# Cryptum169/another-cuda-sift

Hardware: AMD Instinct MI355X
Metric: detectAndCompute Mpix/s + 2kx2k 128-D match ms at 1/2/4/8 MI355X (higher is better)
Workload: dtype f32; 1 GPU; C2: detectAndCompute on 1920x1200 frames, 16 per step per GPU (one launch per stage for the batch), numOctaveLayers=3 (5 DoG scales/octave), numOctaves=3, upscale=false, numFeatures=5000; frames HBM-resident; frames_per_launch=16, streams_per_gpu=2, parallelism=frame-sharded x1, no data-path collective, descriptor_mode=fixed-point (default), keypoints_per_frame=4366

## Files before the change

### another-cuda-sift_amd/csrc/detector.hip

```cpp
#include <hip/hip_runtime.h>

#include <algorithm>
#include <cmath>
#include <cstdio>

#include "detector_state.h"

namespace sift_amd {
namespace det {

thread_local std::string g_err;

int fail(int code, const std::string& msg) {
    g_err = msg;
    return code;
}

namespace {

int gaussian_ntaps(double sigma) { return (int)lrint(sigma * 4 * 2 + 1) | 1; }

Taps gaussian_taps(double sigma) {
    Taps t{};
    const int n = gaussian_ntaps(sigma);
// ... 101 lines not shown
            snprintf(msg, sizeof msg,
                     "sigma %g with numOctaveLayers %d gives a layer blur of one tap (its sigma %g < 0.0625); "
                     "the smallest kernel has 3 taps",
                     d->cfg.sigma, L, sig[i]);
            return fail(SIFT_HIP_ERR_INVALID, msg);
        }
    d->initTaps = gaussian_taps((double)sig_diff);
    d->layerTaps.assign(L + 3, Taps{});
    for (int i = 1; i < L + 3; i++) d->layerTaps[i] = gaussian_taps(sig[i]);
    d->tailOct = L + 3 <= kTailMaxPlanes ? tail_first_octave(d->pyr, d->layerTaps.data(), L) : d->nOct;
    d->threshold = (float)(int)std::floor(0.5 * d->cfg.contrastThreshould / L * 255 * 1.0);
    d->kp.contrastThreshold = (float)d->cfg.contrastThreshould;
    d->kp.edgeThreshold = (float)d->cfg.edgeThreshould;
    d->kp.sigma = (float)d->cfg.sigma;
    d->kp.numFeatures = d->cfg.numFeatures;
    double sumPx = 0;
    for (int o = 0; o < d->nOct; o++) sumPx += (double)d->pyr.oct[o].W * d->pyr.oct[o].H;
    auto clampu = [](double v, double lo, double hi) { return (unsigned)std::max(lo, std::min(v, hi)); };
    d->capCand = clampu(sumPx * L / 8, 16384, 1u << 20);
    d->kp.capRefined = std::min(d->capCand, 1u << 18);
    d->kp.capOriented = 2 * d->kp.capRefined;
    const int nfeat = d->cfg.numFeatures;
    d->kp.capFinal = d->cfg.maxKeypoints > 0 ? (unsigned)d->cfg.maxKeypoints
                     : nfeat > 0             ? clampu(nfeat + std::max(nfeat / 4, 512), 1024, 65536)
                                             : clampu(sumPx / 32, 4096, 65536);
    const double sclMax = d->cfg.sigma * std::pow(2.0, (L + 0.5) / L);
    d->kp.oriRmax = (int)lrint(4.5 * sclMax) + 1;
    d->kp.descRmax = std::min((int)lrint(3.0 * sclMax * 1.4142135623730951 * 2.5) + 1, 60);
    const double hw = 3.0 * sclMax;
    d->kp.descNrec = std::min((int)std::ceil((5.0 * hw + 3.0) * (5.0 * hw + 3.0)), 8192);
    return SIFT_HIP_OK;
}

void upload_exp_tab() {
    const double A0 = .9670371139572337719125840413672004409288e-2;
    float tab[64];
    for (int j = 0; j < 64; j++) tab[j] = (float)(std::exp2((double)j / 64.0) * A0);
    upload_exp_table(tab);
    upload_desc_exp_table(tab);
}

void bind_lane(sift_hip_detector* d, int k, int idx) {
    Lane& L = d->lanes[k];
    const ArenaLayout& a = d->lay;
    char* A = L.arena;
    d->ln = k;
    d->stream = L.stream;
    d->dInput = reinterpret_cast<float*>(A + a.input);
    d->dUp = d->firstOctave < 0 ? reinterpret_cast<float*>(A + a.up) : nullptr;
    d->dPyr = reinterpret_cast<float*>(A + a.pyr);
    for (int o = 0; o < d->nOct; o++) d->pyr.oct[o].base = d->dPyr + a.octave[o];
    d->dCand = reinterpret_cast<uint2*>(A + a.cand);
    d->dRef = reinterpret_cast<RefKpt*>(A + a.ref);
    d->dOri = reinterpret_cast<OriKpt*>(A + a.ori);
    d->dSlot = reinterpret_cast<int*>(A + a.slot);
    d->dOrder = reinterpret_cast<int*>(A + a.order);
    d->dJobs = reinterpret_cast<DescJob*>(A + a.jobs);
    d->dJord = reinterpret_cast<JobOrder*>(A + a.jord);
    d->dRange = reinterpret_cast<unsigned*>(A + a.range);
    d->dBcount = reinterpret_cast<unsigned*>(A + a.bcount);
    d->dBoff = reinterpret_cast<unsigned*>(A + a.boff);
    d->dBitmap = reinterpret_cast<uint32_t*>(A + a.bitmap);
    d->dCtr = reinterpret_cast<Counters*>(A + a.ctr);
    char* R = A + (size_t)idx * d->afs;
    for (int b = 0; b < d->kSlots; b++) {
        d->dKpts3[b] = reinterpret_cast<float*>(R + a.k3[b]);
        d->dFeats4[b] = reinterpret_cast<float*>(R + a.f4[b]);
        d->dDesc[b] = reinterpret_cast<uint16_t*>(R + a.desc[b]);
        d->dSide[b] = Sidecar{reinterpret_cast<int8_t*>(R + a.codes[b]), reinterpret_cast<int*>(R + a.ckeys[b])};
    }
    d->hCtr = L.hCtr + idx;
    d->hCtrDev = L.hCtrDev + idx;
}

const uint16_t* frame_desc(const sift_hip_detector* d, long long f) {
    const auto& r = d->frecs[f & (kFrameRing - 1)];
    return reinterpret_cast<const uint16_t*>(d->lanes[r.lane].arena + (size_t)r.idx * d->afs + d->lay.desc[r.slot]);
}
const Counters& frame_counters(const sift_hip_detector* d, long long f, int i) {
    const auto& r = d->frecs[f & (kFrameRing - 1)];
    return d->lanes[r.lane].hCtr[(size_t)r.slot * d->lanes[r.lane].B + r.idx + i];
}

int allocate(sift_hip_detector* d) {
    HIPCHK(hipSetDevice(d->device));
    d->allocated = true;
    if (d->tailOct < d->nOct) {
        int optin = 0;
        if (hipDeviceGetAttribute(&optin, hipDeviceAttributeSharedMemPerBlockOptin, d->device) != hipSuccess ||
            optin < (int)(sizeof(float) * kTailLdsFloats) || tail_init() != hipSuccess) {
            (void)hipGetLastError();
            d->tailOct = d->nOct;
        }
    }
    HIPCHK(hipEventCreateWithFlags(&d->evIn, hipEventDisableTiming));
    HIPCHK(hipEventCreateWithFlags(&d->evOut, hipEventDisableTiming));
    const int W = d->cfg.col_width, H = d->cfg.row_width;
    d->inPitch = (W + 63) / 64 * 64;
    if (d->firstOctave < 0) d->upPitch = (2 * W + 63) / 64 * 64;
    size_t pyrFloats = 0;
    for (int o = 0; o < d->nOct; o++) pyrFloats += (size_t)d->pyr.oct[o].planeStride * (d->L + 3);
    const unsigned capO = d->kp.capOriented, capF = d->kp.capFinal;

    size_t off = 0;
    auto take = [&](size_t bytes) {
        const size_t o = off;
        off += (std::max<size_t>(bytes, 1) + 255) & ~(size_t)255;
        return o;
    };
    ArenaLayout& a = d->lay;
    a.input = take(sizeof(float) * (size_t)d->inPitch * H);
    a.up = d->firstOctave < 0 ? take(sizeof(float) * (size_t)d->upPitch * 2 * H) : 0;
    a.pyr = take(sizeof(float) * pyrFloats);
    a.cand = take(sizeof(uint2) * d->capCand);
    a.ref = take(sizeof(RefKpt) * d->kp.capRefined);
    a.ori = take(sizeof(OriKpt) * capO);
    a.slot = take(sizeof(int) * capO);
    a.order = take(sizeof(int) * capO);
    a.jobs = take(sizeof(DescJob) * capF);
    a.jord = take(sizeof(JobOrder));
    a.range = take(sizeof(unsigned) * 2 * 2 * kRangeSlots);
    a.bcount = take(sizeof(unsigned) * (size_t)d->kp.numBuckets);
    a.boff = take(sizeof(unsigned) * (size_t)d->kp.numBuckets);
    a.bitmap = take(sizeof(uint32_t) * d->bitmapWords);
    a.ctr = take(sizeof(Counters));
    for (int b = 0; b < d->kSlots; b++) {
        a.k3[b] = take(sizeof(float) * 3 * (size_t)capF);
        a.f4[b] = take(sizeof(float) * 4 * (size_t)capF);
        a.desc[b] = take(sizeof(uint16_t) * 128 * (size_t)capF);
        a.codes[b] = take(128 * (size_t)capF);
        a.ckeys[b] = take(sizeof(int) * (size_t)capF);
    }
    d->afs = (long)off;
    upload_exp_tab();
    return SIFT_HIP_OK;
}

int build_graphs(sift_hip_detector* d);

int add_lane(sift_hip_detector* d, int B, int nslots) {
    if (d->nLanes >= kMaxLanes) return fail(SIFT_HIP_ERR_STATE, "no lane left");
    const int k = d->nLanes;
    Lane& L = d->lanes[k];
    d->nLanes++;
    L.B = B;
    L.nslots = nslots;
    HIPCHK(hipStreamCreateWithFlags(&L.stream, hipStreamNonBlocking));
    if (hipMalloc((void**)&L.arena, (size_t)d->afs * B) != hipSuccess)
        return fail(SIFT_HIP_ERR_NOMEM, "hipMalloc of the frame arenas failed");
    HIPCHK(hipMemsetAsync(L.arena, 0, (size_t)d->afs * B, L.stream));
    const size_t nh = (size_t)nslots * B;
    HIPCHK(hipHostMalloc((void**)&L.hCtr, sizeof(Counters) * nh, hipHostMallocMapped | hipHostMallocCoherent));
    memset(L.hCtr, 0, sizeof(Counters) * nh);
    HIPCHK(hipHostGetDevicePointer((void**)&L.hCtrDev, L.hCtr, 0));
    if (hipMalloc((void**)&L.dHostTab, sizeof(char*) * nh) != hipSuccess)
        return fail(SIFT_HIP_ERR_NOMEM, "hipMalloc of the host results table failed");
    HIPCHK(hipMemsetAsync(L.dHostTab, 0, sizeof(char*) * nh, L.stream));
    for (int b = 0; b < d->kSlots; b++) {
        HIPCHK(hipEventCreateWithFlags(&L.evFrame[b], hipEventDisableTiming));
        HIPCHK(hipEventRecord(L.evFrame[b], L.stream));
    }
    std::fill(std::begin(L.hostFrame), std::end(L.hostFrame), -1LL);
    const size_t inBytes = sizeof(float) * (size_t)d->inPitch * d->cfg.row_width;
    for (int i = 0; i < Lane::kInSlots; i++) {
        HIPCHK(hipHostMalloc(&L.hStage[i], inBytes, hipHostMallocMapped | hipHostMallocNonCoherent));
        HIPCHK(hipEventCreateWithFlags(&L.evRead[i], hipEventDisableTiming));
        HIPCHK(hipEventRecord(L.evRead[i], L.stream));
    }
    bind_lane(d, k);
    for (int i = 0; i < B; i++)
        for (int b = 0; b < d->kSlots; b++)
            register_sidecar(d, fptr(d->dDesc[b], (long)i * d->afs),
                             Sidecar{fptr(d->dSide[b].codes, (long)i * d->afs), fptr(d->dSide[b].keys, (long)i * d->afs)},
                             (int)d->kp.capFinal);
    if (d->hostWant)
        if (int rc = ensure_host_res(d, L)) return rc;
    if (int rc = build_graphs(d)) return rc;
    L.ready = true;
    return SIFT_HIP_OK;
}

unsigned* range_keys(sift_hip_detector* d, int p) { return d->dRange + (size_t)p * 2 * kRangeSlots; }

void enqueue_head(sift_hip_detector* d, const void* img, int pitch, int fmt, int parity, int nf, long sfs) {
    const int W = d->cfg.col_width, H = d->cfg.row_width;
    const bool u8 = fmt == SIFT_HIP_U8;
    const Frames fr{nf, d->afs};
    const double inB = (double)W * H * (u8 ? 1 : 4) * nf;
    if (d->firstOctave < 0) {
        d->timed("upsample", inB + (double)W * H * 16 * nf, [&] {
            if (u8)
                launch_upsample2x_u8((const uint8_t*)img, pitch, W, H, d->dUp, d->upPitch, fr, sfs, d->stream);
            else
                launch_upsample2x((const float*)img, pitch, W, H, d->dUp, d->upPitch, fr, sfs, d->stream);
        });
    } else {
        const OctGeom& g = d->pyr.oct[0];
        d->timed("blur_init", inB + (double)W * H * 4 * nf, [&] {
            long s = sfs;
            if (u8) {
                if (launch_blur_u8((const uint8_t*)img, pitch, W, H, g.base, g.pitch, d->initTaps, fr, sfs, d->stream,
                                   range_keys(d, parity), d->dCtr))
                    return;
                launch_u8_to_f32((const uint8_t*)img, pitch, W, H, d->dInput, d->inPitch, fr, sfs, d->stream);
                img = d->dInput;
                pitch = d->inPitch;
                s = d->afs;
            }
            launch_blur((const float*)img, pitch, W, H, g.base, g.pitch, DecOut{}, d->initTaps, fr, s, d->stream,
                        range_keys(d, parity), d->dCtr);
        });
    }
}

void left_tail(sift_hip_detector* d, int nf, hipStream_t s) {
    if (d->tailOct >= d->nOct) return;
    double bytes = 0;
    for (int o = d->tailOct; o < d->nOct; o++)
        bytes += (double)d->pyr.oct[o].W * d->pyr.oct[o].H * 4 * (o == d->tailOct ? 1 + (d->L + 2) : (d->L + 2)) * nf;
    d->timed("pyr_tail", bytes, [&] { launch_blur_tail(d->pyr, d->layerTaps.data(), d->L, d->tailOct, Frames{nf, d->afs}, s); });
}

void enqueue_pyramid(sift_hip_detector* d, int nf, int parity) {
    hipStream_t s = d->stream;
    const int L = d->L;
    const Frames fr{nf, d->afs};
    if (d->firstOctave < 0) {
        const OctGeom& g = d->pyr.oct[0];
        d->timed("blur_init", (double)g.W * g.H * 8 * nf, [&] {
            launch_blur(d->dUp, d->upPitch, g.W, g.H, g.base, g.pitch, DecOut{}, d->initTaps, fr, d->afs, s,
                        range_keys(d, parity), d->dCtr);
        });
    }
    static const char* blurNames[kMaxOctaves] = {"blur_o0", "blur_o1", "blur_o2", "blur_o3", "blur_o4", "blur_o5",
                                                 "blur_o6", "blur_o7", "blur_o8", "blur_o9", "blur_o10", "blur_o11",
                                                 "blur_o12", "blur_o13", "blur_o14", "blur_o15"};
    struct Job {
        int o, i;
        BlurDesc b;
        double bytes;
    };
    std::vector<Job> jobs;
    for (int o = 0; o < d->tailOct; o++) {
        const OctGeom& g = d->pyr.oct[o];
        for (int i = 1; i < L + 3; i++) {
            Job j{o, i, {}, 0};
            j.b.src = g.base + (size_t)(i - 1) * g.planeStride;
            j.b.spitch = g.pitch;
            j.b.dst = g.base + (size_t)i * g.planeStride;
            j.b.dpitch = g.pitch;
            j.b.W = g.W;
            j.b.H = g.H;
            j.b.taps = &d->layerTaps[i];
            j.bytes = (double)g.W * g.H * 8 * nf;
            if (i == L && o + 1 < d->nOct) {
                const OctGeom& n = d->pyr.oct[o + 1];
                j.b.dec = DecOut{n.base, n.pitch, n.W, n.H};
                j.bytes += (double)n.W * n.H * 4 * nf;
            }
            jobs.push_back(j);
        }
    }
    auto idx = [&](int o, int i) { return o * (L + 2) + (i - 1); };
    std::vector<bool> done(jobs.size(), false);
    auto ready = [&](size_t k) {
        const Job& j = jobs[k];
        if (done[k]) return false;
        if (j.i >= 2) return (bool)done[idx(j.o, j.i - 1)];
        return j.o == 0 || (bool)done[idx(j.o - 1, L)];
    };
    if (jobs.empty()) left_tail(d, nf, s);
    for (size_t left = jobs.size(); left > 0;) {
        int a = -1, b = -1;
        for (size_t k = 0; k < jobs.size() && b < 0; k++)
            if (ready(k)) (a < 0 ? a : b) = (int)k;
        const Job& ja = jobs[a];
        bool paired = false;
        if (b >= 0) {
            const Job& jb = jobs[b];
            char name[16];
            snprintf(name, sizeof name, "blur_o%d+o%d", ja.o, jb.o);
            d->timed(name, ja.bytes + jb.bytes, [&] { paired = launch_blur_pair(ja.b, jb.b, fr, s); });
            if (paired) {
                done[b] = true;
                left--;
            }
        }
        if (!paired) {
            d->timed(blurNames[ja.o], ja.bytes, [&] {
                launch_blur(ja.b.src, ja.b.spitch, ja.b.W, ja.b.H, ja.b.dst, ja.b.dpitch, ja.b.dec,
                            *ja.b.taps, fr, d->afs, s);
            });
        }
        done[a] = true;
        left--;
    }
    if (!jobs.empty()) left_tail(d, nf, s);
}

void enqueue_extrema(sift_hip_detector* d, int nf) {
    hipStream_t s = d->stream;
    const int L = d->L;
    const Frames fr{nf, d->afs};
    double exBytes = 0;
    for (int o = 0; o < d->nOct; o++) exBytes += (double)d->pyr.oct[o].W * d->pyr.oct[o].H * 4 * (L + 3) * nf;
    d->timed("extrema", exBytes, [&] {
        if (!launch_extrema_all(d->pyr, d->threshold, d->dCand, d->dCtr, d->capCand, fr, s))
            for (int o = 0; o < d->nOct; o++)
                launch_extrema(d->pyr, o, d->threshold, d->dCand, d->dCtr, d->capCand, fr, s);
    });
}

void enqueue_refine(sift_hip_detector* d, int nf) {
    const Frames fr{nf, d->afs};
    d->timed("refine", 0, [&] {
        launch_refine(d->pyr, d->dCand, d->capCand, d->dCtr, d->dBitmap, d->dRef, d->kp, fr, d->stream);
    });
}

void enqueue_orientation(sift_hip_detector* d, int nf, const MaskArg& mask) {
    const Frames fr{nf, d->afs};
    d->timed("orientation", 0,
             [&] { launch_orientation(d->pyr, d->dRef, d->dCtr, d->dOri, d->dBitmap, d->kp, fr, d->stream, mask); });
}

void enqueue_order(sift_hip_detector* d, int slot, int nf, const MaskArg& mask) {
    hipStream_t s = d->stream;
    const int parity = slot & 1;
    const Frames fr{nf, d->afs};
    if (d->kp.numBuckets <= kOrderMaxBuckets) {
        d->timed("order", 0, [&] {
            launch_order(d->pyr, d->dOri, d->dCtr, range_keys(d, parity ^ 1), d->dBcount, d->dBoff, d->dSlot, d->dOrder,
                         d->dJord, d->kp, fr, s, mask);
        });
    } else {
        d->timed("select", 0, [&] { launch_select(d->dOri, d->dCtr, range_keys(d, parity ^ 1), d->kp, fr, s); });
        d->timed("bucket_count", 0,
                 [&] { launch_bucket_count(d->dOri, d->dCtr, d->dBcount, d->dSlot, d->kp, fr, s, mask); });
        d->timed("bucket_scan", 0, [&] { launch_bucket_scan(d->dBcount, d->dBoff, d->dCtr, d->kp, fr, s); });
        d->timed("bucket_scatter", 0,
                 [&] { launch_bucket_scatter(d->dOri, d->dCtr, d->dBoff, d->dSlot, d->dOrder, d->kp, fr, s); });
    }
    d->timed("bucket_rank", 0, [&] {
        if (d->kp.numBuckets <= kOrderMaxBuckets)
            launch_rank_final(d->pyr, d->dOri, d->dBcount, d->dBoff, d->dOrder, d->dCtr, d->dJord, d->dJobs, d->dKpts3[slot],
                              d->dFeats4[slot], d->kp, fr, s);
        else
            launch_bucket_rank(d->pyr, d->dOri, d->dBcount, d->dBoff, d->dOrder, d->dCtr, d->dJobs, d->dKpts3[slot],
                               d->dFeats4[slot], d->kp, fr, s);
    });
}

void enqueue_descriptor(sift_hip_detector* d, int slot, int nf) {
    const Frames fr{nf, d->afs};
    d->timed("descriptor", 0, [&] {
        launch_descriptor(d->dJobs, d->dCtr, range_keys(d, slot & 1), d->dDesc[slot], d->dSide[slot],
                          d->hCtrDev + (size_t)slot * d->lane().B,
                          HostOut{d->lane().dHostTab + (size_t)slot * d->lane().B, d->dKpts3[slot], d->dFeats4[slot],
                                  d->kp.capFinal},
                          d->kp, fr, d->stream);
    });
}

void enqueue_provided(sift_hip_detector* d, int slot, const ProvidedKpt* kpts, int n) {
    d->timed("provided_jobs", (double)n * (sizeof(ProvidedKpt) + sizeof(DescJob) + 28), [&] {
        launch_provided_jobs(d->pyr, kpts, n, d->cfg.col_width, d->cfg.row_width, d->dCtr, range_keys(d, (slot & 1) ^ 1),
                             d->dJobs, d->dKpts3[slot], d->dFeats4[slot], d->stream);
    });
}

void enqueue_body(sift_hip_detector* d, int slot, int nf, const MaskArg& mask = MaskArg{}) {
    enqueue_pyramid(d, nf, slot & 1);
    enqueue_extrema(d, nf);
    enqueue_refine(d, nf);
    enqueue_orientation(d, nf, mask);
    enqueue_order(d, slot, nf, mask);
    enqueue_descriptor(d, slot, nf);
}

void head_node(sift_hip_detector* d, HeadNode& h, const float* img, int pitch, int parity, int nf, long sfs) {
    const int W = d->cfg.col_width, H = d->cfg.row_width;
    const Frames fr{nf, d->afs};
    if (d->firstOctave < 0) {
        head_upsample_node(h, img, pitch, W, H, d->dUp, d->upPitch, fr, sfs);
    } else {
        const OctGeom& g = d->pyr.oct[0];
        head_blur_node(h, img, pitch, W, H, g.base, g.pitch, d->initTaps, fr, sfs, range_keys(d, parity), d->dCtr);
    }
}

int capture(sift_hip_detector* d, int slot, int nf, FrameGraph& G) {
    hipGraph_t body = nullptr;
    HIPCHK(hipStreamBeginCapture(d->stream, hipStreamCaptureModeThreadLocal));
    enqueue_body(d, slot, nf);
    HIPCHK(hipStreamEndCapture(d->stream, &body));
    HIPCHK(hipGraphInstantiate(&G.exec, body, nullptr, nullptr, 0));
    HIPCHK(hipGraphDestroy(body));
    G.in = HeadIn{d->dInput, d->inPitch, d->afs};
    HIPCHK(hipStreamBeginCapture(d->stream, hipStreamCaptureModeThreadLocal));
    enqueue_head(d, G.in.img, G.in.pitch, SIFT_HIP_F32, slot & 1, nf, G.in.sfs);
    enqueue_body(d, slot, nf);
    HIPCHK(hipStreamEndCapture(d->stream, &G.graphH));
    size_t nroot = 0;
    HIPCHK(hipGraphGetRootNodes(G.graphH, nullptr, &nroot));
    if (nroot != 1) return fail(SIFT_HIP_ERR_RUNTIME, "captured frame graph: expected one root (the head)");
    HIPCHK(hipGraphGetRootNodes(G.graphH, &G.head, &nroot));
    hipGraphNodeType ty;
    HIPCHK(hipGraphNodeGetType(G.head, &ty));
    if (ty != hipGraphNodeTypeKernel) return fail(SIFT_HIP_ERR_RUNTIME, "captured frame graph: the head is not a kernel");
    HIPCHK(hipGraphInstantiate(&G.execH, G.graphH, nullptr, nullptr, 0));
    return SIFT_HIP_OK;
}

int build_graphs(sift_hip_detector* d) {
    Lane& L = d->lane();
    for (int b = 0; b < L.nslots; b++)
        for (int kind = 0; kind < (L.B > 1 ? 2 : 1); kind++)
            if (int rc = capture(d, b, kind == 0 ? L.B : 1, L.graphs[b][kind])) return rc;
    return SIFT_HIP_OK;
}

bool event_done(hipEvent_t e) {
    const hipError_t r = hipEventQuery(e);
    if (r == hipSuccess) return true;
    (void)hipGetLastError();
    return false;
}

int warm_lane(sift_hip_detector* d) {
    Lane& L = d->lane();
    const int kinds = L.B > 1 ? 2 : 1;
    for (int kind = 0; kind < kinds; kind++)
        for (int b = 0; b < L.nslots; b++) {
            HIPCHK(hipGraphLaunch(L.graphs[b][kind].execH, L.stream));
            HIPCHK(hipEventRecord(L.evFrame[b], L.stream));
            L.nfOf[b] = kind == 0 ? L.B : 1;
        }
    L.launched = (long long)kinds * L.nslots;
    return SIFT_HIP_OK;
}

int run_frame(sift_hip_detector* d, const FrameJob& job) {
    const void* img = job.img;
    const int pitch = job.pitch, fmt = job.fmt, nf = job.nf;
    const long long f = d->submitted;
    Lane& L = d->lane();
    const int slot = (int)(L.launched % L.nslots);
    const bool compute = job.nProvided >= 0;
    const bool dump = !d->dgDir.empty() && nf == 1 && d->firstFrame > 0 && !compute;
    const int W = d->cfg.col_width, H = d->cfg.row_width;
    if (dump) {
        if (!d->dDg && hipMalloc((void**)&d->dDg, sizeof(float) * (size_t)W * H) != hipSuccess)
            return fail(SIFT_HIP_ERR_NOMEM, "hipMalloc of the stage-dump input failed");
        if (fmt == SIFT_HIP_U8)
            launch_u8_to_f32((const uint8_t*)img, pitch, W, H, d->dDg, W, Frames{1, 0}, 0, d->stream);
        else
            HIPCHK(hipMemcpy2DAsync(d->dDg, sizeof(float) * W, img, sizeof(float) * (size_t)pitch, sizeof(float) * W,
                                    H, hipMemcpyDefault, d->stream));
    }
    const bool replay = d->useGraph && !d->timing && !compute && !job.mask.p;
    FrameGraph* G = replay ? L.graph(slot, nf) : nullptr;
    if (G && fmt == SIFT_HIP_F32 && event_done(L.evFrame[slot])) {
        const HeadIn in{img, pitch, job.sfs};
        if (!(G->in == in)) {
            HeadNode& h = d->headNode;
            head_node(d, h, static_cast<const float*>(img), pitch, slot & 1, nf, job.sfs);
            HIPCHK(hipGraphExecKernelNodeSetParams(G->execH, G->head, &h.p));
            G->in = in;
        }
        HIPCHK(hipGraphLaunch(G->execH, d->stream));
    } else {
        enqueue_head(d, img, pitch, fmt, slot & 1, nf, job.sfs);
        if (G) {
            HIPCHK(hipGraphLaunch(G->exec, d->stream));
        } else if (compute) {
            enqueue_pyramid(d, 1, slot & 1);
            enqueue_provided(d, slot, job.provided, job.nProvided);
            enqueue_descriptor(d, slot, 1);
        } else {
            enqueue_body(d, slot, nf, job.mask);
        }
    }
    HIPCHK(hipEventRecord(L.evFrame[slot], d->stream));
    const int nums = job.numbered ? nf : 1;
    L.nfOf[slot] = nf;
    L.slotFrame[slot] = f;
    L.slotNum[slot] = nums;
    L.launched++;
    L.last = f + nums - 1;
    for (int i = 0; i < nums; i++) d->frec(f + i) = sift_hip_detector::FrameRec{d->ln, slot, i};
    for (int i = 0; i < nf; i++) sidecar_refreshed(fptr(d->dDesc[slot], (long)i * d->afs));
    d->submitted = f + nums;
    if (dump) {
        HIPCHK(hipStreamSynchronize(d->stream));
        if (d->timing) d->collect_timing();
        d->current = f;
        d->curLane = d->ln;
        d->curIdx = 0;
        d->cur = slot;
        complete_counts(d);
        return dump_stage_files(d);
    }
    return SIFT_HIP_OK;
}

void make_current(sift_hip_detector* d, long long f) {
    d->current = f;
    d->curLane = d->frec(f).lane;
    d->curIdx = d->frec(f).idx;
    d->cur = d->frec(f).slot;
    d->countsValid = false;
    bind_lane(d, d->curLane, d->curIdx);
}

void complete_counts(sift_hip_detector* d) {
    const long long f = d->current;
    auto n = [&](long long g) {
        return g < d->firstFrame ? 0 : (int)std::min<unsigned>(frame_counters(d, g).final_n, d->kp.capFinal);
    };
    d->count = n(f);
    d->prevCount = n(f - 1);
    d->countsValid = true;
}

int ensure_counts(sift_hip_detector* d) {
    if (d->countsValid) return SIFT_HIP_OK;
    for (long long g : {d->current - 1, d->current})
        if (g >= d->firstFrame) {
            const auto& r = d->frec(g);
            HIPCHK(hipEventSynchronize(d->lanes[r.lane].evFrame[r.slot]));
        }
    complete_counts(d);
    return SIFT_HIP_OK;
}

int sync_lanes(sift_hip_detector* d) {
    for (int k = 0; k < d->nLanes; k++)
        if (d->lanes[k].ready) HIPCHK(hipStreamSynchronize(d->lanes[k].stream));
    if (d->timing) d->collect_timing();
    return SIFT_HIP_OK;
}

int finish_frame(sift_hip_detector* d) {
    if (int rc = run_group(d)) return rc;
    if (int rc = sync_lanes(d)) return rc;
    if (d->submitted > 0) {
        make_current(d, d->submitted - 1);
        complete_counts(d);
    }
    return SIFT_HIP_OK;
}

}
}

void sift_amd::set_last_error(const std::string& msg) { det::g_err = msg; }

int batch_frames_of(sift_hip_detector* d) {
    if (d->current < d->firstFrame) return 0;
    const Lane& L = d->lane();
    return L.slotNum[d->cur] > 1 ? 1 : L.nfOf[d->cur];
}

#define CHECK_HANDLE(h)                                                                       \
    do {                                                                                      \
        if (!(h)) return fail(SIFT_HIP_ERR_INVALID, "null handle");                          \
        if (!(h)->allocated || !(h)->lanes[0].ready)                                          \
            return fail(SIFT_HIP_ERR_STATE, "sift_hip_warmup not called");                    \
        HIPCHK(hipSetDevice((h)->device));                                                    \
        bind_lane((h), (h)->curLane, (h)->curIdx);                                            \
    } while (0)

static int bind_counts_if_warm(sift_hip_detector* d) {
    if (!d->allocated || !d->lanes[0].ready) return SIFT_HIP_OK;
    HIPCHK(hipSetDevice(d->device));
    bind_lane(d, d->curLane, d->curIdx);
    return ensure_counts(d);
}

static const Counters& current_counters(sift_hip_detector* d, int i = 0) {
    return d->hCtr[(size_t)d->cur * d->lane().B + i];
}

static int copy_results_d2h(sift_hip_detector* d, int slot, long off, int n, float* k3, float* f4, uint16_t* desc) {
    hipStream_t s;
    if (int rc = copy_stream(d, &s)) return rc;
    HIPCHK(hipStreamWaitEvent(s, d->lane().evFrame[slot], 0));
    if (n > 0) {
        if (k3) HIPCHK(hipMemcpyAsync(k3, fptr(d->dKpts3[slot], off), sizeof(float) * 3 * n, hipMemcpyDeviceToHost, s));
        if (f4) HIPCHK(hipMemcpyAsync(f4, fptr(d->dFeats4[slot], off), sizeof(float) * 4 * n, hipMemcpyDeviceToHost, s));
        if (desc)
            HIPCHK(hipMemcpyAsync(desc, fptr(d->dDesc[slot], off), sizeof(uint16_t) * 128 * n, hipMemcpyDeviceToHost, s));
    }
    HIPCHK(hipStreamSynchronize(s));
    return SIFT_HIP_OK;
}

static int want_host_results(sift_hip_detector* d, bool desc) {
    if (!d->hostWant)
        for (int k = 0; k < d->nLanes; k++)
            if (d->lanes[k].ready)
                if (int rc = ensure_host_res(d, d->lanes[k])) return rc;
    d->hostWant = std::max(d->hostWant, desc ? 2 : 1);
    return SIFT_HIP_OK;
}

static bool region_holds_current(const sift_hip_detector* d, const Lane& L, int region, bool desc) {
    return L.hostFrame[region] == d->current && d->current >= d->firstFrame && (!desc || L.hostDesc[region]);
// ... 589 lines not shown
```

### another-cuda-sift_amd/csrc/extrema.hip

```cpp
#include "sift_kernels.h"
#include "sift_math.h"

namespace sift_amd {

constexpr int EX_TW = 64;
constexpr int EX_TH = 16;
constexpr int EX_SW = EX_TW + 2;
constexpr int EX_SH = EX_TH + 2;
constexpr int EX_LIST = 512;

template <bool FLAT>
__global__ __launch_bounds__(256) void k_extrema(OctGeom g, int L, int o, float thr, uint2* __restrict__ cand,
                                                 Counters* __restrict__ ctr, unsigned cap, long fs) {
    extern __shared__ float dog[];
    g.base = fptr(g.base, blockIdx.z * fs);
    cand = fptr(cand, blockIdx.z * fs);
    ctr = fptr(ctr, blockIdx.z * fs);
    const int tid = threadIdx.x;
    const int tile = xcd_tile(blockIdx.y * gridDim.x + blockIdx.x, gridDim.x * gridDim.y);
    const int x0 = (tile % gridDim.x) * EX_TW, y0 = (tile / gridDim.x) * EX_TH;
    const int W = g.W, H = g.H, pitch = g.pitch;
    constexpr int PS = EX_SH * EX_SW;
    __shared__ unsigned s_cnt, s_base;
    __shared__ uint2 s_list[EX_LIST];
    if (tid == 0) s_cnt = 0;

    for (int i = tid; i < PS; i += 256) {
        const int ly = i / EX_SW, lx = i - ly * EX_SW;
        const int gy = y0 - 1 + ly, gx = x0 - 1 + lx;
        if (gy >= 0 && gy < H && gx >= 0 && gx < W) {
            const float* p = g.base + (size_t)gy * pitch + gx;
            float prev = p[0];
            for (int d = 0; d < L + 2; d++) {
                const float next = p[(size_t)(d + 1) * g.planeStride];
                dog[d * PS + i] = next - prev;
                prev = next;
            }
        } else {
            for (int d = 0; d < L + 2; d++) dog[d * PS + i] = 0.f;
        }
    }
    __syncthreads();

    const int lane = tid & 63;
    const int total = EX_TH * EX_TW * L;
    for (int base = 0; base < total; base += 256) {
        const int i = base + tid;
        bool hit = false;
        int layer = 0, r = 0, c = 0;
        if (i < total) {
            layer = 1 + i / (EX_TH * EX_TW);
            const int rem = i - (layer - 1) * (EX_TH * EX_TW);
            const int ly = rem >> 6, lx = rem & 63;
            r = y0 + ly;
            c = x0 + lx;
            if (r >= 5 && r < H - 5 && c >= 5 && c < W - 5) {
                const float* cur = dog + layer * PS + (ly + 1) * EX_SW + (lx + 1);
                const float val = cur[0];
                if (fabsf(val) > thr) {
                    hit = true;
                    if constexpr (FLAT) {
                        hit = false;
#pragma unroll
                        for (int dy = -1; dy <= 1; dy++)
#pragma unroll
                            for (int dx = -1; dx <= 1; dx++) hit |= val != cur[dy * EX_SW + dx];
                    }
                    if (val > 0) {
#pragma unroll
                        for (int d = -1; d <= 1; d++)
#pragma unroll
                            for (int dy = -1; dy <= 1; dy++)
#pragma unroll
                                for (int dx = -1; dx <= 1; dx++) hit &= val >= cur[d * PS + dy * EX_SW + dx];
                    } else {
#pragma unroll
                        for (int d = -1; d <= 1; d++)
#pragma unroll
                            for (int dy = -1; dy <= 1; dy++)
#pragma unroll
                                for (int dx = -1; dx <= 1; dx++) hit &= val <= cur[d * PS + dy * EX_SW + dx];
                    }
                }
            }
        }
        const unsigned long long mask = __ballot(hit);
        if (mask) {
            unsigned basepos = 0;
            if (lane == 0) basepos = atomicAdd(&s_cnt, (unsigned)__popcll(mask));
            basepos = __shfl(basepos, 0);
            if (hit) {
                const unsigned pos = basepos + (unsigned)__popcll(mask & ((1ull << lane) - 1ull));
                const uint2 q = make_uint2((unsigned)(o << 8 | layer), (unsigned)(r << 16 | c));
                if (pos < EX_LIST) {
                    s_list[pos] = q;
                } else {
                    const unsigned gp = atomicAdd(&ctr->cand, 1u);
                    if (gp < cap)
                        cand[gp] = q;
                    else
                        atomicOr(&ctr->overflow, 1u);
                }
            }
        }
    }
    __syncthreads();
    const unsigned nl = min(s_cnt, (unsigned)EX_LIST);
    if (tid == 0) s_base = nl ? atomicAdd(&ctr->cand, nl) : 0u;
    __syncthreads();
    for (unsigned k = tid; k < nl; k += 256) {
        const unsigned pos = s_base + k;
        if (pos < cap)
            cand[pos] = s_list[k];
        else
            atomicOr(&ctr->overflow, 1u);
    }
}

constexpr int EX4_LIST = 2048;
constexpr int kExCpl = 4;
constexpr int EX4_COLS = 64 * kExCpl;

template <int LT, bool FLAT, int EX4_TR, int EX4_AHEAD, int NB = 1, int CPL = kExCpl>
__device__ __forceinline__ void extrema_block(const OctGeom& g, int o, float thr, uint2* __restrict__ cand,
                                              Counters* __restrict__ ctr, unsigned cap, int tile, int strips,
                                              uint2* s_list, unsigned& s_cnt, unsigned& s_base) {
    constexpr int NG = LT + 3, ND = LT + 2;
    static_assert(CPL * LT <= 31 && (CPL == 2 || CPL == 4), "hit bits per row");
    static_assert(NB == 1 || (EX4_TR % 3 == 0 && EX4_TR % (EX4_AHEAD + 1) == 0),
                  "multi-step streams: the ring and the load sets repeat every EX4_TR rows");
    typedef float f4 __attribute__((ext_vector_type(CPL)));
    constexpr int EX4_COLS = 64 * CPL;
    constexpr int TR = EX4_TR * NB;
    const int tid = threadIdx.x, lane = tid & 63, wave = tid >> 6;
    const int x0 = (tile % strips) * EX4_COLS, y0 = ((tile / strips) * 4 + wave) * TR;
    const int W = g.W, H = g.H, pitch = g.pitch;
    const int xl = x0 + CPL * lane;
    const int xe = min(max(lane == 0 ? x0 - 1 : x0 + EX4_COLS, 0), W - 1);
    const __amdgpu_buffer_rsrc_t rsrc = __builtin_amdgcn_make_buffer_rsrc(
        g.base, 0, (int)min((long)NG * g.planeStride * 4, 0x7fffffffL), 0x00020000);
    if (tid == 0) s_cnt = 0;
    __syncthreads();

    bool colOK[CPL];
#pragma unroll
    for (int c = 0; c < CPL; c++) colOK[c] = xl + c >= 5 && xl + c < W - 5;

    f4 rd[3][ND];
    float re[3][ND];
    f4 rv[EX4_AHEAD + 1][NG];
    float rev[EX4_AHEAD + 1][NG];
#if defined(SIFT_EX_DIAG) && (SIFT_EX_DIAG == 1 || SIFT_EX_DIAG == 3)
    const bool l4 = xl < W, le = false;
#else
    const bool l4 = xl < W, le = lane == 0 || lane == 63;
#endif
    auto issue_row = [&](int y, f4 (&v)[NG], float (&e)[NG]) {
#if defined(SIFT_EX_DIAG) && (SIFT_EX_DIAG == 2 || SIFT_EX_DIAG == 3)
        y = min(max(y, y0), y0 + TR - 1);
#endif
        const int yc = min(max(y, 0), H - 1);
        const unsigned off4 = l4 ? (unsigned)(yc * pitch + xl) * 4u : 0x80000000u;
        const unsigned offe = le ? (unsigned)(yc * pitch + xe) * 4u : 0x80000000u;
#pragma unroll
        for (int d = 0; d < NG; d++) {
            const int so = (int)((long)d * g.planeStride * 4);
            if constexpr (CPL == 4)
                v[d] = __builtin_bit_cast(f4, __builtin_amdgcn_raw_buffer_load_b128(rsrc, off4, so, 0));
            else
                v[d] = __builtin_bit_cast(f4, __builtin_amdgcn_raw_buffer_load_b64(rsrc, off4, so, 0));
            e[d] = __builtin_bit_cast(float, __builtin_amdgcn_raw_buffer_load_b32(rsrc, offe, so, 0));
        }
    };
    auto emit_row = [&](int r, unsigned hits) {
        if (!__ballot(hits != 0)) return;
        const unsigned cnt = (unsigned)__popc(hits);
        unsigned excl = 0, tot = 0;
#pragma unroll
        for (int b = 0; b < 5; b++) {
            const unsigned long long bm = __ballot((cnt >> b) & 1u);
            excl += __builtin_amdgcn_mbcnt_hi((unsigned)(bm >> 32), __builtin_amdgcn_mbcnt_lo((unsigned)bm, 0u)) << b;
            tot += (unsigned)__popcll(bm) << b;
        }
        unsigned base = 0;
        if (lane == 0) base = atomicAdd(&s_cnt, tot);
        unsigned pos = __builtin_amdgcn_readfirstlane(base) + excl;
        for (unsigned m = hits; m; m &= m - 1u, pos++) {
            const int f = __builtin_ctz(m), l = f / CPL + 1, c = f % CPL;
            const uint2 q = make_uint2((unsigned)(o << 8 | l), (unsigned)(r << 16 | (xl + c)));
            if (pos < EX4_LIST) {
                s_list[pos] = q;
            } else {
                const unsigned gp = atomicAdd(&ctr->cand, 1u);
                if (gp < cap)
                    cand[gp] = q;
                else
                    atomicOr(&ctr->overflow, 1u);
            }
        }
    };
    auto test_row = [&](int r, int A, int B, int C) -> unsigned {
        const bool rowOK = r >= 5 && r < H - 5;
        f4 hx[ND], hn[ND];
#pragma unroll
        for (int d = 0; d < ND; d++) {
            f4 vx, vn;
#pragma unroll
            for (int c = 0; c < CPL; c++) {
                vx[c] = fmaxf(fmaxf(rd[A][d][c], rd[B][d][c]), rd[C][d][c]);
                vn[c] = fminf(fminf(rd[A][d][c], rd[B][d][c]), rd[C][d][c]);
            }
            const float ex = fmaxf(fmaxf(re[A][d], re[B][d]), re[C][d]);
            const float en = fminf(fminf(re[A][d], re[B][d]), re[C][d]);
            const float lx = dpp_left_or(ex, vx[CPL - 1]), ln = dpp_left_or(en, vn[CPL - 1]);
            const float rx = dpp_right_or(ex, vx[0]), rn = dpp_right_or(en, vn[0]);
#pragma unroll
            for (int c = 0; c < CPL; c++) {
                const float xa = c == 0 ? lx : vx[c - 1], xb = c == CPL - 1 ? rx : vx[c + 1];
                const float na = c == 0 ? ln : vn[c - 1], nb = c == CPL - 1 ? rn : vn[c + 1];
                hx[d][c] = fmaxf(fmaxf(xa, vx[c]), xb);
                hn[d][c] = fminf(fminf(na, vn[c]), nb);
            }
        }
        unsigned hits = 0;
#pragma unroll
        for (int l = 1; l <= LT; l++)
#pragma unroll
            for (int c = 0; c < CPL; c++) {
                const float v = rd[B][l][c];
                const float M = fmaxf(fmaxf(hx[l - 1][c], hx[l][c]), hx[l + 1][c]);
                const float m = fminf(fminf(hn[l - 1][c], hn[l][c]), hn[l + 1][c]);
                bool h = rowOK && colOK[c] && fabsf(v) > thr && v == (v > 0 ? M : m);
                if constexpr (FLAT) h = h && hx[l][c] != hn[l][c];
                hits |= (unsigned)h << ((l - 1) * CPL + c);
            }
        return hits;
    };

    if (y0 < H) {
        constexpr int NS = EX4_AHEAD + 1;
        const int nsteps = NB == 1 ? 1 : min(NB, (min(H - 5, y0 + TR) - y0 + EX4_TR - 1) / EX4_TR);
        const int nr = nsteps * EX4_TR + 2, yb = y0 + nsteps * EX4_TR;
        const bool up = (wave & 1) != 0;
        auto strip_row = [&](int m) { return up ? yb - m : y0 - 1 + m; };
        auto tested_row = [&](int k) { return up ? yb - 1 - k : y0 + k; };
        auto form = [&](int m, int km, f4 (&d4)[ND], float (&de)[ND]) {
#pragma unroll
            for (int d = 0; d < ND; d++) {
                d4[d] = rv[km][d + 1] - rv[km][d];
                de[d] = rev[km][d + 1] - rev[km][d];
            }
            if (m + NS < nr) issue_row(strip_row(m + NS), rv[km], rev[km]);
        };
#pragma unroll
        for (int m = 0; m < NS; m++) issue_row(strip_row(m), rv[m], rev[m]);
        form(0, 0, rd[0], re[0]);
        form(1, 1 % NS, rd[1], re[1]);
#pragma unroll 1
        for (int kb = 0; kb < nsteps * EX4_TR; kb += EX4_TR) {
#pragma unroll
            for (int k6 = 0; k6 < EX4_TR; k6++) {
                const int k = kb + k6;
                const int A = k6 % 3, B = (k6 + 1) % 3, C = (k6 + 2) % 3;
                form(k + 2, (k6 + 2) % NS, rd[C], re[C]);
                const int r = tested_row(k);
                emit_row(r, test_row(r, A, B, C));
            }
        }
    }
    __syncthreads();
    const unsigned nl = min(s_cnt, (unsigned)EX4_LIST);
    if (tid == 0) s_base = nl ? atomicAdd(&ctr->cand, nl) : 0u;
    __syncthreads();
    for (unsigned k = tid; k < nl; k += 256) {
        const unsigned pos = s_base + k;
        if (pos < cap)
            cand[pos] = s_list[k];
        else
            atomicOr(&ctr->overflow, 1u);
    }
}

constexpr int kExTallMin = 2048;
constexpr int kExStream = 2;
struct ExtremaPlan {
    int start[kMaxOctaves + 1];
    int strips[kMaxOctaves];
    int tall[kMaxOctaves];
};

template <int LT, bool FLAT>
__global__ __launch_bounds__(256) void k_extrema_all(PyrDesc pyr, ExtremaPlan plan, float thr,
                                                     uint2* __restrict__ cand, Counters* __restrict__ ctr,
                                                     unsigned cap, long fs) {
    __shared__ unsigned s_cnt, s_base;
    __shared__ uint2 s_list[EX4_LIST];
    const int per = plan.start[pyr.nOct];
    const int t = xcd_tile(blockIdx.x, gridDim.x);
    const int f = t / per, b = t - f * per;
    int o = 0;
    while (o + 1 < pyr.nOct && b >= plan.start[o + 1]) o++;
    OctGeom g = pyr.oct[o];
    g.base = fptr(g.base, f * fs);
    cand = fptr(cand, f * fs);
    ctr = fptr(ctr, f * fs);
    const int blk = b - plan.start[o];
    if (plan.tall[o])
        extrema_block<LT, FLAT, 6, 2, kExStream>(g, o, thr, cand, ctr, cap, blk, plan.strips[o], s_list, s_cnt, s_base);
    else
        extrema_block<LT, FLAT, 2, 2>(g, o, thr, cand, ctr, cap, blk, plan.strips[o], s_list, s_cnt, s_base);
}

void launch_extrema(const PyrDesc& pyr, int o, float threshold, uint2* cand, Counters* ctr, unsigned cap,
                    const Frames& fr, hipStream_t s) {
    const OctGeom& g = pyr.oct[o];
    dim3 grid((g.W + EX_TW - 1) / EX_TW, (g.H + EX_TH - 1) / EX_TH, fr.nf);
    const size_t lds = sizeof(float) * (size_t)(pyr.L + 2) * EX_SH * EX_SW;
    if (threshold == 0.f)
        hipLaunchKernelGGL((k_extrema<true>), grid, dim3(256), lds, s, g, pyr.L, o, threshold, cand, ctr, cap,
                           fr.stride);
    else
        hipLaunchKernelGGL((k_extrema<false>), grid, dim3(256), lds, s, g, pyr.L, o, threshold, cand, ctr, cap,
                           fr.stride);
}

bool launch_extrema_all(const PyrDesc& pyr, float threshold, uint2* cand, Counters* ctr, unsigned cap,
                        const Frames& fr, hipStream_t s) {
    if (pyr.L < 1 || pyr.L > 6) return false;
    ExtremaPlan plan{};
    int total = 0;
    for (int o = 0; o < pyr.nOct; o++) {
        const OctGeom& g = pyr.oct[o];
        const int strips = (g.W + EX4_COLS - 1) / EX4_COLS;
        const bool tall = strips * ((g.H + 5) / 6) * fr.nf >= (fr.nf > 1 ? 1024 : kExTallMin);
        const int tr = tall ? 6 * kExStream : 2;
        plan.start[o] = total;
        plan.strips[o] = strips;
        plan.tall[o] = tall;
        total += strips * ((g.H + 4 * tr - 1) / (4 * tr));
    }
    plan.start[pyr.nOct] = total;
    const bool flat = threshold == 0.f;
    switch (pyr.L) {
#define SIFT_EX_CASE(LV) \
    case LV: {                                                                                                      \
        if (flat)                                                                                                   \
            hipLaunchKernelGGL((k_extrema_all<LV, true>), dim3(total * fr.nf), dim3(256), 0, s, pyr, plan, threshold, \
                               cand, ctr, cap, fr.stride);                                                          \
        else                                                                                                        \
            hipLaunchKernelGGL((k_extrema_all<LV, false>), dim3(total * fr.nf), dim3(256), 0, s, pyr, plan,         \
                               threshold, cand, ctr, cap, fr.stride);                                               \
        break;                                                                                                      \
    }
        SIFT_EX_CASE(1)
        SIFT_EX_CASE(2)
        SIFT_EX_CASE(3)
        SIFT_EX_CASE(4)
        SIFT_EX_CASE(5)
        SIFT_EX_CASE(6)
#undef SIFT_EX_CASE
    }
    return true;
}

}
```

Baseline: 30140 Mpix/s.

## Stream only inner Gaussian planes in extrema and verify outer DoG neighbours lazily

```diff
diff --git a/another-cuda-sift_amd/csrc/detector.hip b/another-cuda-sift_amd/csrc/detector.hip
--- a/another-cuda-sift_amd/csrc/detector.hip
+++ b/another-cuda-sift_amd/csrc/detector.hip
@@ -427,8 +427,9 @@
     hipStream_t s = d->stream;
     const int L = d->L;
     const Frames fr{nf, d->afs};
+    const int planes = L <= 6 ? L + 1 : L + 3;
     double exBytes = 0;
-    for (int o = 0; o < d->nOct; o++) exBytes += (double)d->pyr.oct[o].W * d->pyr.oct[o].H * 4 * (L + 3) * nf;
+    for (int o = 0; o < d->nOct; o++) exBytes += (double)d->pyr.oct[o].W * d->pyr.oct[o].H * 4 * planes * nf;
     d->timed("extrema", exBytes, [&] {
         if (!launch_extrema_all(d->pyr, d->threshold, d->dCand, d->dCtr, d->capCand, fr, s))
             for (int o = 0; o < d->nOct; o++)
diff --git a/another-cuda-sift_amd/csrc/extrema.hip b/another-cuda-sift_amd/csrc/extrema.hip
--- a/another-cuda-sift_amd/csrc/extrema.hip
+++ b/another-cuda-sift_amd/csrc/extrema.hip
@@ -124,8 +124,8 @@
 template <int LT, bool FLAT, int EX4_TR, int EX4_AHEAD, int NB = 1, int CPL = kExCpl>
 __device__ __forceinline__ void extrema_block(const OctGeom& g, int o, float thr, uint2* __restrict__ cand,
                                               Counters* __restrict__ ctr, unsigned cap, int tile, int strips,
-                                              uint2* s_list, unsigned& s_cnt, unsigned& s_base) {
-    constexpr int NG = LT + 3, ND = LT + 2;
+                                              uint2* s_list, unsigned& s_cnt, unsigned& s_keep, unsigned& s_base) {
+    constexpr int NG = LT + 3, NP = LT + 1, ND = LT;
     static_assert(CPL * LT <= 31 && (CPL == 2 || CPL == 4), "hit bits per row");
     static_assert(NB == 1 || (EX4_TR % 3 == 0 && EX4_TR % (EX4_AHEAD + 1) == 0),
                   "multi-step streams: the ring and the load sets repeat every EX4_TR rows");
@@ -139,7 +139,7 @@
     const int xe = min(max(lane == 0 ? x0 - 1 : x0 + EX4_COLS, 0), W - 1);
     const __amdgpu_buffer_rsrc_t rsrc = __builtin_amdgcn_make_buffer_rsrc(
         g.base, 0, (int)min((long)NG * g.planeStride * 4, 0x7fffffffL), 0x00020000);
-    if (tid == 0) s_cnt = 0;
+    if (tid == 0) s_cnt = s_keep = 0;
     __syncthreads();
 
     bool colOK[CPL];
@@ -148,14 +148,14 @@
 
     f4 rd[3][ND];
     float re[3][ND];
-    f4 rv[EX4_AHEAD + 1][NG];
-    float rev[EX4_AHEAD + 1][NG];
+    f4 rv[EX4_AHEAD + 1][NP];
+    float rev[EX4_AHEAD + 1][NP];
 #if defined(SIFT_EX_DIAG) && (SIFT_EX_DIAG == 1 || SIFT_EX_DIAG == 3)
     const bool l4 = xl < W, le = false;
 #else
     const bool l4 = xl < W, le = lane == 0 || lane == 63;
 #endif
-    auto issue_row = [&](int y, f4 (&v)[NG], float (&e)[NG]) {
+    auto issue_row = [&](int y, f4 (&v)[NP], float (&e)[NP]) {
 #if defined(SIFT_EX_DIAG) && (SIFT_EX_DIAG == 2 || SIFT_EX_DIAG == 3)
         y = min(max(y, y0), y0 + TR - 1);
 #endif
@@ -163,14 +163,63 @@
         const unsigned off4 = l4 ? (unsigned)(yc * pitch + xl) * 4u : 0x80000000u;
         const unsigned offe = le ? (unsigned)(yc * pitch + xe) * 4u : 0x80000000u;
 #pragma unroll
-        for (int d = 0; d < NG; d++) {
-            const int so = (int)((long)d * g.planeStride * 4);
+        for (int d = 0; d < NP; d++) {
+            const int so = (int)((long)(d + 1) * g.planeStride * 4);
             if constexpr (CPL == 4)
                 v[d] = __builtin_bit_cast(f4, __builtin_amdgcn_raw_buffer_load_b128(rsrc, off4, so, 0));
             else
                 v[d] = __builtin_bit_cast(f4, __builtin_amdgcn_raw_buffer_load_b64(rsrc, off4, so, 0));
             e[d] = __builtin_bit_cast(float, __builtin_amdgcn_raw_buffer_load_b32(rsrc, offe, so, 0));
         }
+    };
+    auto outer_ok = [&](bool have, int l, unsigned rc) -> bool {
+        const unsigned ps4 = (unsigned)(g.planeStride * 4);
+        const unsigned at = (unsigned)((int)(rc >> 16) * pitch + (int)(rc & 0xffffu)) * 4u;
+        constexpr unsigned kPast = 0x90000000u;
+        constexpr int NO = LT == 1 ? 2 : 1;
+        const bool prov = have && (l == 1 || l == LT);
+        unsigned lo[NO];
+        if constexpr (LT == 1) {
+            lo[0] = at;
+            lo[1] = at + 2u * ps4;
+        } else {
+            lo[0] = at + (l == 1 ? 0u : (unsigned)(LT + 1) * ps4);
+        }
+        auto ld = [&](unsigned off) {
+            return __builtin_bit_cast(float, __builtin_amdgcn_raw_buffer_load_b32(rsrc, off, 0, 0));
+        };
+        auto rows = [&](bool on, const int (&DY)[2], int ndy, float& mx, float& mn) {
+            float a[NO][2][3], b[NO][2][3];
+#pragma unroll
+            for (int n = 0; n < NO; n++)
+#pragma unroll
+                for (int j = 0; j < ndy; j++)
+#pragma unroll
+                    for (int dx = 0; dx < 3; dx++) {
+                        const unsigned off = on ? lo[n] + (unsigned)(DY[j] * pitch + dx - 1) * 4u : kPast;
+                        a[n][j][dx] = ld(off);
+                        b[n][j][dx] = ld(off + ps4);
+                    }
+            mx = mn = b[0][0][0] - a[0][0][0];
+#pragma unroll
+            for (int n = 0; n < NO; n++)
+#pragma unroll
+                for (int j = 0; j < ndy; j++)
+#pragma unroll
+                    for (int dx = 0; dx < 3; dx++) {
+                        const float dv = b[n][j][dx] - a[n][j][dx];
+                        mx = fmaxf(mx, dv);
+                        mn = fminf(mn, dv);
+                    }
+        };
+        const unsigned vo = prov ? at + (unsigned)l * ps4 : kPast;
+        const float v0 = ld(vo), v1 = ld(vo + ps4);
+        float mx, mn;
+        rows(prov, {0, 0}, 1, mx, mn);
+        const float v = v1 - v0;
+        const bool in = prov && (v > 0 ? mx <= v : mn >= v);
+        rows(in, {-1, 1}, 2, mx, mn);
+        return !prov || (in && (v > 0 ? mx <= v : mn >= v));
     };
     auto emit_row = [&](int r, unsigned hits) {
         if (!__ballot(hits != 0)) return;
@@ -190,7 +239,7 @@
             const uint2 q = make_uint2((unsigned)(o << 8 | l), (unsigned)(r << 16 | (xl + c)));
             if (pos < EX4_LIST) {
                 s_list[pos] = q;
-            } else {
+            } else if (outer_ok(true, l, q.y)) {
                 const unsigned gp = atomicAdd(&ctr->cand, 1u);
                 if (gp < cap)
                     cand[gp] = q;
@@ -227,11 +276,12 @@
         for (int l = 1; l <= LT; l++)
 #pragma unroll
             for (int c = 0; c < CPL; c++) {
-                const float v = rd[B][l][c];
-                const float M = fmaxf(fmaxf(hx[l - 1][c], hx[l][c]), hx[l + 1][c]);
-                const float m = fminf(fminf(hn[l - 1][c], hn[l][c]), hn[l + 1][c]);
+                const float v = rd[B][l - 1][c];
+                float M = hx[l - 1][c], m = hn[l - 1][c];
+                if (l > 1) M = fmaxf(M, hx[l - 2][c]), m = fminf(m, hn[l - 2][c]);
+                if (l < LT) M = fmaxf(M, hx[l][c]), m = fminf(m, hn[l][c]);
                 bool h = rowOK && colOK[c] && fabsf(v) > thr && v == (v > 0 ? M : m);
-                if constexpr (FLAT) h = h && hx[l][c] != hn[l][c];
+                if constexpr (FLAT) h = h && hx[l - 1][c] != hn[l - 1][c];
                 hits |= (unsigned)h << ((l - 1) * CPL + c);
             }
         return hits;
@@ -269,13 +319,29 @@
         }
     }
     __syncthreads();
+    static_assert(EX4_LIST <= 65536 && kMaxOctaves <= 256, "slot and o << 8 | l share a word");
     const unsigned nl = min(s_cnt, (unsigned)EX4_LIST);
-    if (tid == 0) s_base = nl ? atomicAdd(&ctr->cand, nl) : 0u;
+    for (unsigned k0 = 0; k0 < nl; k0 += 256) {
+        const unsigned k = k0 + tid;
+        const bool have = k < nl;
+        const uint2 q = have ? s_list[k] : make_uint2(0u, 0u);
+        const bool keep = outer_ok(have, (int)(q.x & 0xffu), q.y) && have;
+        const unsigned long long km = __ballot(keep);
+        unsigned base = 0;
+        if (lane == 0 && km) base = atomicAdd(&s_keep, (unsigned)__popcll(km));
+        const unsigned slot = __builtin_amdgcn_readfirstlane(base) +
+                              __builtin_amdgcn_mbcnt_hi((unsigned)(km >> 32), __builtin_amdgcn_mbcnt_lo((unsigned)km, 0u));
+        if (have) s_list[k].x = keep ? q.x | slot << 16 : ~0u;
+    }
+    __syncthreads();
+    if (tid == 0) s_base = s_keep ? atomicAdd(&ctr->cand, s_keep) : 0u;
     __syncthreads();
     for (unsigned k = tid; k < nl; k += 256) {
-        const unsigned pos = s_base + k;
+        const uint2 q = s_list[k];
+        if (q.x == ~0u) continue;
+        const unsigned pos = s_base + (q.x >> 16);
         if (pos < cap)
-            cand[pos] = s_list[k];
+            cand[pos] = make_uint2(q.x & 0xffffu, q.y);
         else
             atomicOr(&ctr->overflow, 1u);
     }
@@ -293,7 +359,7 @@
 __global__ __launch_bounds__(256) void k_extrema_all(PyrDesc pyr, ExtremaPlan plan, float thr,
                                                      uint2* __restrict__ cand, Counters* __restrict__ ctr,
                                                      unsigned cap, long fs) {
-    __shared__ unsigned s_cnt, s_base;
+    __shared__ unsigned s_cnt, s_keep, s_base;
     __shared__ uint2 s_list[EX4_LIST];
     const int per = plan.start[pyr.nOct];
     const int t = xcd_tile(blockIdx.x, gridDim.x);
@@ -306,9 +372,9 @@
     ctr = fptr(ctr, f * fs);
     const int blk = b - plan.start[o];
     if (plan.tall[o])
-        extrema_block<LT, FLAT, 6, 2, kExStream>(g, o, thr, cand, ctr, cap, blk, plan.strips[o], s_list, s_cnt, s_base);
+        extrema_block<LT, FLAT, 6, 2, kExStream>(g, o, thr, cand, ctr, cap, blk, plan.strips[o], s_list, s_cnt, s_keep, s_base);
     else
-        extrema_block<LT, FLAT, 2, 2>(g, o, thr, cand, ctr, cap, blk, plan.strips[o], s_list, s_cnt, s_base);
+        extrema_block<LT, FLAT, 2, 2>(g, o, thr, cand, ctr, cap, blk, plan.strips[o], s_list, s_cnt, s_keep, s_base);
 }
 
 void launch_extrema(const PyrDesc& pyr, int o, float threshold, uint2* cand, Counters* ctr, unsigned cap,
```

New measurement: 31480 Mpix/s (median of 6 runs). +4.5%, better.
